# SAP/nested-hashing-psi

Hardware: AMD Instinct MI355X
Metric: server PIE ciphertexts/sec (higher is better)
Workload: dtype u64

## Files before the change

### nested_hashing_psi_amd/csrc/kernels_pie.hip

```cpp
#include <stdlib.h>

#include <cassert>

#include <algorithm>

#include "kernels.hpp"
#include "madasm.h"
#include "stage_a_common.h"
#include "pie_arith.h"

namespace piehip {

static const u32 TPB = 256;

typedef u64 u64x2 __attribute__((ext_vector_type(2)));


template <int BPT>
__global__ void __launch_bounds__(TPB) stage_a_kernel(const DevConsts *__restrict__ dc, u32 N, u32 L, u32 K, u32 b, u32 E,
                                                      const u64 *__restrict__ idx, const u64 *__restrict__ minus,
                                                      const u64 *__restrict__ db, u64 *__restrict__ acc, u32 bstride, u32 h0,
                                                      u32 nq, u32 q)
{
    const u32 n = 2 * (blockIdx.x * TPB + threadIdx.x);
    const u32 l = blockIdx.y;
    const u32 groups = b / BPT;
    const u32 h = h0 + blockIdx.z / groups, beta0 = (blockIdx.z % groups) * BPT;
    if (n >= N) return;
    const Mod m = dc->mod[l];
    const size_t LN = (size_t)L * N;
    const u64 *pi = idx + ((size_t)h * E) * 2 * LN + (size_t)l * N + n;
    const u64 *pd = db + (((size_t)h * bstride + beta0) * E) * LN + (size_t)l * N + n;
    const size_t bin_stride = (size_t)E * LN;
    U128 a[BPT][2][2];
#pragma unroll
    for (int t = 0; t < BPT; t++)
#pragma unroll
        for (int c = 0; c < 2; c++) a[t][c][0] = a[t][c][1] = U128{0, 0};
    for (u32 j = 0; j < E; j++) {
        const u64x2 i0 = *reinterpret_cast<const u64x2 *>(pi + (size_t)j * 2 * LN);
        const u64x2 i1 = *reinterpret_cast<const u64x2 *>(pi + (size_t)j * 2 * LN + LN);
        u64x2 d[BPT];
#pragma unroll
        for (int t = 0; t < BPT; t++) {
            typedef u64 u64v2 __attribute__((ext_vector_type(2)));
            const u64v2 v = __builtin_nontemporal_load(reinterpret_cast<const u64v2 *>(pd + (size_t)t * bin_stride + (size_t)j * LN));
            d[t].x = v.x, d[t].y = v.y;
        }
#pragma unroll
        for (int t = 0; t < BPT; t++) {
            mac128(a[t][0][0], i0.x, d[t].x);
            mac128(a[t][0][1], i0.y, d[t].y);
            mac128(a[t][1][0], i1.x, d[t].x);
            mac128(a[t][1][1], i1.y, d[t].y);
        }
        if ((j & 31) == 31) {
#pragma unroll
            for (int t = 0; t < BPT; t++)
#pragma unroll
                for (int c = 0; c < 2; c++)
#pragma unroll
                    for (int e = 0; e < 2; e++) a[t][c][e] = U128{reduce128(a[t][c][e], m), 0};
        }
    }
    const u64x2 m0 = *reinterpret_cast<const u64x2 *>(minus + (size_t)l * N + n);
    const u64x2 m1 = *reinterpret_cast<const u64x2 *>(minus + LN + (size_t)l * N + n);
#pragma unroll
    for (int t = 0; t < BPT; t++) {
        u64 *po = acc + ((((size_t)(beta0 + t) * nq + q) * K + h) * 2) * LN + (size_t)l * N + n;
        u64x2 r0, r1;
        r0.x = addmod(reduce128(a[t][0][0], m), m0.x, m.q);
        r0.y = addmod(reduce128(a[t][0][1], m), m0.y, m.q);
        r1.x = addmod(reduce128(a[t][1][0], m), m1.x, m.q);
        r1.y = addmod(reduce128(a[t][1][1], m), m1.y, m.q);
        *reinterpret_cast<u64x2 *>(po) = r0;
        *reinterpret_cast<u64x2 *>(po + LN) = r1;
    }
}

static const int SA_DEPTH = 4;
template <int BPT>
__global__ void __launch_bounds__(TPB) stage_a_mad_kernel(const DevConsts *__restrict__ dc, u32 N, u32 L, u32 K, u32 b, u32 E,
                                                          const u64 *__restrict__ idx, const u64 *__restrict__ minus,
                                                          const u64 *__restrict__ db, u64 *__restrict__ acc, u32 bstride, u32 h0,
                                                          u32 nq, u32 q, StageAXOut xo)
{
    const u32 nl = threadIdx.x;
    const u32 n = blockIdx.x * TPB + nl;
    const u32 l = blockIdx.y;
    const u32 groups = b / BPT;
    const u32 h = h0 + blockIdx.z / groups, beta0 = (blockIdx.z % groups) * BPT;
    if (n >= N) return;
    const Mod m = dc->mod[l];
    const size_t LN = (size_t)L * N;
    const u64 *pi = idx + ((size_t)h * E) * 2 * LN + (size_t)l * N + blockIdx.x * TPB;
    const u64 *pd = db + (((size_t)h * bstride + beta0) * E) * LN + (size_t)l * N + blockIdx.x * TPB;
    const size_t bin_stride = (size_t)E * LN;
    ColAcc a[BPT][2];
#pragma unroll
    for (int t = 0; t < BPT; t++) a[t][0] = a[t][1] = ColAcc{0, 0, 0};
    auto load_term = [&](u32 j, u64 (&vi)[2], u64 (&vd)[BPT]) {
        const u64 *pij = pi + (size_t)j * 2 * LN, *pdj = pd + (size_t)j * LN;
        vi[0] = pij[nl];
        vi[1] = (pij + LN)[nl];
#pragma unroll
        for (int t = 0; t < BPT; t++) vd[t] = __builtin_nontemporal_load(pdj + (size_t)t * bin_stride + nl);
    };
    u64 qiv[SA_DEPTH][2], qdv[SA_DEPTH][BPT];
#pragma unroll
    for (int d = 0; d < SA_DEPTH; d++)
        if ((u32)d < E) load_term(d, qiv[d], qdv[d]);
    auto term = [&](u32 j, u64 (&vi)[2], u64 (&vd)[BPT]) {
        const Split30 i0 = split30(vi[0]), i1 = split30(vi[1]);
#pragma unroll
        for (int t = 0; t < BPT; t++) colacc_mac2(a[t][0], a[t][1], i0, i1, vd[t]);
        if (j + SA_DEPTH < E) load_term(j + SA_DEPTH, vi, vd);
        if ((j % COLACC_MAX_TERMS) == COLACC_MAX_TERMS - 1 && j + 1 < E) {
#pragma unroll
            for (int t = 0; t < BPT; t++) colacc_carry(a[t][0]), colacc_carry(a[t][1]);
        }
        if ((j % COLACC_MAX_TOTAL) == COLACC_MAX_TOTAL - 1 && j + 1 < E) {
#pragma unroll
            for (int t = 0; t < BPT; t++)
#pragma unroll
                for (int c = 0; c < 2; c++) {
                    const u64 r = reduce124(colacc_value(a[t][c]), m);
                    a[t][c] = ColAcc{r & 0x3FFFFFFFull, r >> 30, 0};
                }
        }
    };
    for (u32 j = 0; j < E; j += SA_DEPTH) {
#pragma unroll
        for (int d = 0; d < SA_DEPTH; d++)
            if (j + d < E) term(j + d, qiv[d], qdv[d]);
    }
    const bool xdir = h == 0 && xo.out != nullptr;
    const u32 noff = n + ((xdir ? ~0u : 0u) & (lane_home(n, xo.logns) - n));
#pragma unroll
    for (int t = 0; t < BPT; t++) {
        const size_t row = (size_t)(beta0 + t) * nq + q;
        u64 *const base = xdir ? xo.out + ((row * 4) * xo.M + l) * N : acc + ((row * K + h) * 2) * LN + (size_t)l * N;
        const size_t cstride = xdir ? (size_t)xo.M * N : LN;
        u64 *const po = base + noff;
#pragma unroll
        for (int c = 0; c < 2; c++)
            po[(size_t)c * cstride] = addmod_nb(colacc_reduce<true>(a[t][c], m, 0 - m.q), minus[(size_t)c * LN + (size_t)l * N + n], m.q);
    }
}

template <int BPT, int Q, int DEPTH>
__global__ void __launch_bounds__(TPB) stage_a_mad_batch_kernel(const DevConsts *__restrict__ dc, u32 N, u32 L, u32 K, u32 b, u32 E,
                                                                StageAQueries qs, const u64 *__restrict__ db, u64 *__restrict__ acc,
                                                                u32 bstride, u32 h0, u32 nq, u32 q0, u32 tiles, StageAXOut xo)
{
    StageATile tl;
    if (!stage_a_tile((N + TPB - 1) / TPB, L, tiles, (b + BPT - 1) / BPT, tl)) return;
    const u32 nl = threadIdx.x, n0 = tl.bx * TPB, l = tl.l, h = h0 + tl.hz, beta0 = tl.grp * BPT;
    const u32 n = n0 + nl;
    if (n >= N) return;
    const u32 tmax = __builtin_amdgcn_readfirstlane(min((u32)BPT, b - beta0) - 1);
    const Mod m = dc->mod[l];
    const size_t LN = (size_t)L * N;
    const size_t ioff = ((size_t)h * E) * 2 * LN + (size_t)l * N + n0;
    const u64 *pd = db + (((size_t)h * bstride + beta0) * E) * LN + (size_t)l * N + n0;
    const size_t bin_stride = (size_t)E * LN;
    StageAAcc<true> a[Q][BPT][2];
    stage_a_terms<BPT, Q, DEPTH, true>(qs, ioff, LN, pd, bin_stride, tmax, nl, E, m, a);
    const bool xdir = h == 0 && xo.out != nullptr;
    const u32 noff = n + ((xdir ? ~0u : 0u) & (lane_home(n, xo.logns) - n));
#pragma unroll
    for (int q = 0; q < Q; q++) {
        u64 mi[2];
#pragma unroll
        for (int c = 0; c < 2; c++) mi[c] = qs.minus[q][(size_t)c * LN + (size_t)l * N + n];
#pragma unroll
        for (int t = 0; t < BPT; t++) {
            if ((u32)t > tmax) continue;
            const size_t row = (size_t)(beta0 + t) * nq + q0 + q;
            u64 *const base = xdir ? xo.out + ((row * 4) * xo.M + l) * N : acc + ((row * K + h) * 2) * LN + (size_t)l * N;
            const size_t cstride = xdir ? (size_t)xo.M * N : LN;
            u64 *const po = base + noff;
#pragma unroll
            for (int c = 0; c < 2; c++) po[(size_t)c * cstride] = addmod_nb(colacc_reduce<true>(a[q][t][c].v, m, 0 - m.q), mi[c], m.q);
        }
    }
}

static void launch_stage_a_uniform(const DevConsts *dc, u32 N, u32 L, u32 K, u32 b, u32 E, const u64 *idx, const u64 *minus,
                                   const u64 *db, u64 *acc, hipStream_t st, bool mad, u32 bstride, u32 h0, u32 hn, int bpt, u32 nq,
                                   u32 q, StageAXOut xo)
{
    const int cpt = mad ? 1 : 2;
    dim3 grid((N / cpt + TPB - 1) / TPB, L, hn * (b / bpt));
#define SA(B_)                                                                                                       \
    do {                                                                                                             \
        if (mad) hipLaunchKernelGGL(stage_a_mad_kernel<B_>, grid, dim3(TPB), 0, st, dc, N, L, K, b, E, idx, minus, db, acc, bstride, h0, nq, q, xo); \
        else hipLaunchKernelGGL(stage_a_kernel<B_>, grid, dim3(TPB), 0, st, dc, N, L, K, b, E, idx, minus, db, acc, bstride, h0, nq, q);  \
    } while (0)
    switch (bpt) {
        case 8: hipLaunchKernelGGL(stage_a_kernel<8>, grid, dim3(TPB), 0, st, dc, N, L, K, b, E, idx, minus, db, acc, bstride, h0, nq, q); break;
        case 7: SA(7); break;
        case 6: SA(6); break;
        case 5: SA(5); break;
        case 4: SA(4); break;
        case 3: SA(3); break;
        case 2: SA(2); break;
        default: SA(1); break;
    }
#undef SA
}

void launch_stage_a(const DevConsts *dc, u32 N, u32 L, u32 K, u32 b, u32 E, const u64 *idx, const u64 *minus,
                    const u64 *db, u64 *acc, hipStream_t st, bool small_moduli, u32 bstride, u32 h0, u32 hn, u32 nq, u32 q,
                    const StageAXOut *xop)
{
    StageAXOut xo;
    if (xop && small_moduli) xo = *xop;
    if (!bstride) bstride = b;
    if (!hn) hn = K - h0;
    if (!nq) nq = 1;
    const bool mad = small_moduli;
    const u32 cap = mad ? 7 : 8;
    u32 bpt = 0;
    for (u32 c = cap; c >= 4; c--)
        if (b % c == 0) {
            bpt = c;
            break;
        }
    if (b <= cap) bpt = b;
    const size_t LN = (size_t)L * N;
    if (bpt) {
        launch_stage_a_uniform(dc, N, L, K, b, E, idx, minus, db, acc, st, mad, bstride, h0, hn, (int)bpt, nq, q, xo);
        return;
    }
    const u32 full = (b / cap) * cap, rest = b - full;
    launch_stage_a_uniform(dc, N, L, K, full, E, idx, minus, db, acc, st, mad, bstride, h0, hn, (int)cap, nq, q, xo);
    StageAXOut xr = xo;
    if (xr.out) xr.out += (size_t)full * nq * 4 * xr.M * N;
    launch_stage_a_uniform(dc, N, L, K, rest, E, idx, minus, db + (size_t)full * E * LN, acc + (size_t)full * nq * K * 2 * LN, st, mad,
                           bstride, h0, hn, (int)rest, nq, q, xr);
}

template <int Q, int BPT>
static void launch_stage_a_batch_qb(const DevConsts *dc, u32 N, u32 L, u32 K, u32 nb, u32 E, const StageAQueries &qs, const u64 *db,
                                    u64 *acc, hipStream_t st, u32 bstride, u32 h0, u32 hn, u32 nq, u32 q0, StageAXOut xo)
{
    const u32 nx = (N + TPB - 1) / TPB;
    constexpr int DEPTH = stage_a_depth(Q, BPT);
    hipLaunchKernelGGL((stage_a_mad_batch_kernel<BPT, Q, DEPTH>), stage_a_grid(nx, L, hn, (nb + BPT - 1) / BPT), dim3(TPB), 0, st, dc, N, L, K,
                       nb, E, qs, db, acc, bstride, h0, nq, q0, nx * L * hn, xo);
}
template <int Q>
static void launch_stage_a_batch_q(const DevConsts *dc, u32 N, u32 L, u32 K, u32 b, u32 E, const StageAQueries &qs, const u64 *db,
                                   u64 *acc, hipStream_t st, u32 bstride, u32 h0, u32 hn, u32 nq, u32 q0, StageAXOut xo)
{
    constexpr u32 cap = stage_a_layer_cap(Q, true);
    const u32 bpt = stage_a_layers(Q, b, cap);
    if constexpr (cap >= 4)
        if (bpt == 4) return launch_stage_a_batch_qb<Q, 4>(dc, N, L, K, b, E, qs, db, acc, st, bstride, h0, hn, nq, q0, xo);
    if constexpr (cap >= 3)
        if (bpt == 3) return launch_stage_a_batch_qb<Q, 3>(dc, N, L, K, b, E, qs, db, acc, st, bstride, h0, hn, nq, q0, xo);
    if (bpt == 2) return launch_stage_a_batch_qb<Q, 2>(dc, N, L, K, b, E, qs, db, acc, st, bstride, h0, hn, nq, q0, xo);
    return launch_stage_a_batch_qb<Q, 1>(dc, N, L, K, b, E, qs, db, acc, st, bstride, h0, hn, nq, q0, xo);
}
void launch_stage_a_batch(const DevConsts *dc, u32 N, u32 L, u32 K, u32 b, u32 E, const StageAQueries &qs, u32 nq, const u64 *db,
                          u64 *acc, hipStream_t st, bool small_moduli, u32 bstride, u32 h0, u32 hn, const StageAXOut *xop)
{
    StageAXOut xo;
    if (xop && small_moduli) xo = *xop;
    if (!bstride) bstride = b;
    if (!hn) hn = K - h0;
    u32 q0 = 0;
    while (small_moduli && nq - q0 >= 2) {
        const u32 g = stage_a_query_group(nq - q0);
        StageAQueries sub = {};
        for (u32 q = 0; q < g; q++) sub.idx[q] = qs.idx[q0 + q], sub.minus[q] = qs.minus[q0 + q];
        if (g == 2) launch_stage_a_batch_q<2>(dc, N, L, K, b, E, sub, db, acc, st, bstride, h0, hn, nq, q0, xo);
        else if (g == 3) launch_stage_a_batch_q<3>(dc, N, L, K, b, E, sub, db, acc, st, bstride, h0, hn, nq, q0, xo);
        else launch_stage_a_batch_q<4>(dc, N, L, K, b, E, sub, db, acc, st, bstride, h0, hn, nq, q0, xo);
        q0 += g;
    }
    for (; q0 < nq; q0++)
        launch_stage_a(dc, N, L, K, b, E, qs.idx[q0], qs.minus[q0], db, acc, st, small_moduli, bstride, h0, hn, nq, q0, xop);
}

#define PIE_ITER_FENCE() __builtin_amdgcn_sched_barrier(0)
typedef const __attribute__((address_space(4))) DevConsts *DcC;
__device__ __forceinline__ DcC dc_iter(const DevConsts *dc)
{
    u64 v = (u64)dc;
    asm volatile("" : "+s"(v));
    return (DcC)v;
}
__device__ __forceinline__ Mod ld_mod(DcC c, u32 i)
{
    Mod m;
    m.q = c->mod[i].q, m.r0 = c->mod[i].r0, m.r1 = c->mod[i].r1, m.n_inv = 0, m.n_inv_sh = 0;
    m.fconst = c->mod[i].fconst, m.fshift = c->mod[i].fshift, m.pad = 0;
    return m;
}

__device__ __forceinline__ void fold_load(const DevConsts *dc, u32 a, u64 u, u64 v, u64 &x0, u64 &x1)
{
    PIE_ITER_FENCE();
    const DcC c = dc_iter(dc);
    const u64 q = c->mod[a].q, nq = neg_u(q);
    x0 = shoup63(u + v, c->fold_ia[a], c->fold_ia_sh[a], nq);
    x1 = shoup63(u + (4 * q - v), c->fold_ib[a], c->fold_ib_sh[a], nq);
}
__device__ __forceinline__ void fold_store(const DevConsts *dc, u32 a, u64 u, u64 v, u64 &y0, u64 &y1)
{
    const DcC c = dc_iter(dc);
    const u64 q = c->mod[a].q;
    const u64 t = shoup63_lazy(v, c->fold_w[a], c->fold_w_sh[a], neg_u(q));
    y0 = u + t;
    y1 = u + (4 * q - t);
}

template <u32 L, bool MAD, bool YIN, int NP, bool LZ = false>
__device__ __forceinline__ void expand_core(const DevConsts *dc, const u64 (&x)[NP][L], u64 (&out)[NP][2 * L + 1])
{
    constexpr u32 Lp = L + 1;
    u64 y[NP][L];
    u64 fsum[NP];
#pragma unroll
    for (int p = 0; p < NP; p++) fsum[p] = 0;
#pragma unroll
    for (u32 i = 0; i < L; i++) {
        PIE_ITER_FENCE();
        const DcC c = dc_iter(dc);
        const Mod mi = ld_mod(c, i);
        const u64 w = c->qhat_inv[i], wsh = c->qhat_inv_sh[i], nq = neg_u(mi.q);
#pragma unroll
        for (int p = 0; p < NP; p++) {
            out[p][i] = x[p][i];
            y[p][i] = YIN ? x[p][i] : mshoup<MAD>(x[p][i], w, wsh, mi.q, nq);
            fsum[p] += mfixfrac<MAD>(y[p][i], mi);
        }
    }
#pragma unroll
    for (u32 j = 0; j < Lp; j++) {
        PIE_ITER_FENCE();
        const DcC c = dc_iter(dc);
        const Mod pj = ld_mod(c, L + j);
        u64 hat[L];
#pragma unroll
        for (u32 i = 0; i < L; i++) hat[i] = c->qhat_modp[i][j];
        const u64 prodmod = c->Q_modp[j], nq = neg_u(pj.q), n2q = neg_u(2 * pj.q);
#pragma unroll
        for (int p = 0; p < NP; p++) out[p][L + j] = crt_out<L, MAD, LZ>(y[p], hat, (fsum[p] + FIX_HALF) >> 60, prodmod, pj, nq, n2q);
    }
}

template <u32 L, bool MAD, bool YIN, int NP, bool LZ = false>
__device__ __forceinline__ void scale_pq_core(const DevConsts *dc, const u64 (&x)[NP][L], u64 (&out)[NP][2 * L + 1])
{
    constexpr u32 Lp = L + 1;
    u64 y[NP][L];
    u64 fsum[NP];
    U128 itot[NP];
#pragma unroll
    for (int p = 0; p < NP; p++) fsum[p] = 0, itot[p] = U128{0, 0};
#pragma unroll
    for (u32 i = 0; i < L; i++) {
        PIE_ITER_FENCE();
        const DcC c = dc_iter(dc);
        const Mod mi = ld_mod(c, i);
        const u64 w = c->qhat_inv[i], wsh = c->qhat_inv_sh[i], pw = c->P_modq[i], pwsh = c->P_modq_sh[i], nq = neg_u(mi.q);
#pragma unroll
        for (int p = 0; p < NP; p++) {
            y[p][i] = YIN ? x[p][i] : mshoup<MAD>(x[p][i], w, wsh, mi.q, nq);
            u64 fl, z;
            mdivmod<MAD>(y[p][i], pw, pwsh, mi.q, nq, fl, z);
            add128(itot[p], U128{fl, 0});
            fsum[p] += mfixfrac<MAD>(z, mi);
        }
    }
    u64 yp[NP][Lp];
    u64 fs2[NP];
#pragma unroll
    for (int p = 0; p < NP; p++) {
        add128(itot[p], U128{(fsum[p] + FIX_HALF) >> 60, 0});
        fs2[p] = 0;
    }
#pragma unroll
    for (u32 j = 0; j < Lp; j++) {
        PIE_ITER_FENCE();
        const DcC c = dc_iter(dc);
        const Mod pj = ld_mod(c, L + j);
        u64 col[L];
#pragma unroll
        for (u32 i = 0; i < L; i++) col[i] = c->PI_modp[i][j];
        const u64 w = c->phat_inv[j], wsh = c->phat_inv_sh[j], nq = neg_u(pj.q);
#pragma unroll
        for (int p = 0; p < NP; p++) {
            u64 r;
            if (MAD) {
                ColAcc a = {itot[p].lo, 0, 0};
#pragma unroll
                for (u32 i = 0; i < L; i++) colacc_mac(a, split30(y[p][i]), split30(col[i]));
                r = LZ ? colacc_reduce123_lazy(a, pj, nq) : colacc_reduce<false>(a, pj, nq);
            } else {
                U128 acc = dot128<L, MAD>(y[p], col);
                add128(acc, itot[p]);
                r = reduce128(acc, pj);
            }
            out[p][L + j] = r;
            yp[p][j] = mshoup<MAD>(r, w, wsh, pj.q, nq);
            fs2[p] += mfixfrac<MAD>(yp[p][j], pj);
        }
    }
#pragma unroll
    for (u32 i = 0; i < L; i++) {
        PIE_ITER_FENCE();
        const DcC c = dc_iter(dc);
        const Mod mi = ld_mod(c, i);
        u64 hat[Lp];
#pragma unroll
        for (u32 j = 0; j < Lp; j++) hat[j] = c->phat_modq[j][i];
        const u64 prodmod = c->P_modq[i], nq = neg_u(mi.q), n2q = neg_u(2 * mi.q);
#pragma unroll
        for (int p = 0; p < NP; p++) out[p][i] = crt_out<Lp, MAD, LZ>(yp[p], hat, (fs2[p] + FIX_HALF) >> 60, prodmod, mi, nq, n2q);
    }
}

template <bool SCALE, bool FOLD, u32 L, bool MAD, bool SKIPQ>
__device__ __forceinline__ void expand_body(const DevConsts *__restrict__ dc, u32 N, const u64 *__restrict__ in, size_t so, size_t si,
                                            u64 *__restrict__ out, u32 out_polys, u32 out_slot, u32 by)
{
    constexpr bool YIN = FOLD && (SCALE || SKIPQ);
    const u32 n = blockIdx.x * TPB + threadIdx.x;
    const u32 H = N / 2;
    if (n >= (FOLD ? H : N)) return;
    const u32 o = by >> 1, c = by & 1;
    constexpr u32 M = 2 * L + 1;
    const u64 *pin = in + (size_t)o * so + (size_t)c * si + n;
    u64 *pout = out + ((size_t)(o * out_polys + out_slot + c) * M) * N + n;
    constexpr int NP = FOLD ? 2 : 1;
    u64 x[NP][L], y[NP][M];
#pragma unroll
    for (u32 i = 0; i < L; i++) {
        if (YIN) {
            PIE_ITER_FENCE();
            const DcC c = dc_iter(dc);
            const u64 q = c->mod[i].q, nq = neg_u(q), u = pin[(size_t)i * N], v = pin[(size_t)i * N + H];
            x[0][i] = shoup63(u + v, c->fold_iaq[i], c->fold_iaq_sh[i], nq);
            x[NP - 1][i] = shoup63(u + (4 * q - v), c->fold_ibq[i], c->fold_ibq_sh[i], nq);
        } else if (FOLD) {
            fold_load(dc, i, pin[(size_t)i * N], pin[(size_t)i * N + H], x[0][i], x[NP - 1][i]);
        } else {
            x[0][i] = pin[(size_t)i * N];
        }
    }
    constexpr bool LZ = FOLD && MAD;
    if (SCALE)
        scale_pq_core<L, MAD, YIN, NP, LZ>(dc, x, y);
    else
        expand_core<L, MAD, YIN, NP, LZ>(dc, x, y);
#pragma unroll
    for (u32 a = 0; a < M; a++) {
        if (!SCALE && a < L && SKIPQ) continue;
        PIE_ITER_FENCE();
        if (FOLD) {
            u64 y0, y1;
            fold_store(dc, a, y[0][a], y[NP - 1][a], y0, y1);
            pout[(size_t)a * N] = y0;
            pout[(size_t)a * N + H] = y1;
        } else {
            pout[(size_t)a * N] = y[0][a];
        }
    }
}

template <bool SCALE, bool FOLD, u32 L, bool MAD, bool SKIPQ>
__global__ void __launch_bounds__(TPB) expand_kernel(const DevConsts *__restrict__ dc, u32 N, const u64 *__restrict__ in,
                                                     size_t so, size_t si, u64 *__restrict__ out, u32 out_polys, u32 out_slot)
{
    expand_body<SCALE, FOLD, L, MAD, SKIPQ>(dc, N, in, so, si, out, out_polys, out_slot, blockIdx.y);
}
template <bool FOLD, u32 L, bool MAD, bool SKIPQ>
__global__ void __launch_bounds__(TPB) expand_both_kernel(const DevConsts *__restrict__ dc, u32 N, const u64 *__restrict__ x, size_t sx,
                                                          const u64 *__restrict__ y, size_t sy, size_t si, u64 *__restrict__ out,
                                                          u32 n_outer)
{
    if (blockIdx.y < 2 * n_outer)
        expand_body<true, FOLD, L, MAD, false>(dc, N, y, sy, si, out, 4, 2, blockIdx.y);
    else
        expand_body<false, FOLD, L, MAD, SKIPQ>(dc, N, x, sx, si, out, 4, 0, blockIdx.y - 2 * n_outer);
}
void launch_expand_both(const DevConsts *dc, u32 N, u32 L, const u64 *x, size_t sx, const u64 *y, size_t sy, size_t si, u32 n_outer,
                        u64 *out, hipStream_t st, bool small_moduli, bool fold, bool skip_q)
{
    dim3 grid(((fold ? N / 2 : N) + TPB - 1) / TPB, n_outer * 4);
#define EB(F_, L_, M_, Q_) hipLaunchKernelGGL((expand_both_kernel<F_, L_, M_, Q_>), grid, dim3(TPB), 0, st, dc, N, x, sx, y, sy, si, out, n_outer)
#define EBL(L_)                                                                          \
    case L_:                                                                             \
        if (fold && small_moduli) { if (skip_q) EB(true, L_, true, true); else EB(true, L_, true, false); }      \
        else if (fold) { if (skip_q) EB(true, L_, false, true); else EB(true, L_, false, false); }                 \
        else if (small_moduli) { if (skip_q) EB(false, L_, true, true); else EB(false, L_, true, false); }       \
        else { if (skip_q) EB(false, L_, false, true); else EB(false, L_, false, false); }                         \
        break;
    switch (L) { EBL(1) EBL(2) EBL(3) EBL(4) EBL(5) EBL(6) EBL(7) }
#undef EBL
#undef EB
}

static void launch_expand_common(bool scale, bool fold, const DevConsts *dc, u32 N, u32 L, const u64 *in, size_t so, size_t si,
                                 u32 n_outer, u64 *out, u32 out_polys, u32 out_slot, hipStream_t st, bool small_moduli, bool skip_q = false)
{
    dim3 grid(((fold ? N / 2 : N) + TPB - 1) / TPB, n_outer * 2);
#define EX(S_, F_, L_, Q_)                                                                                                    \
    do {                                                                                                                      \
        if (small_moduli)                                                                                                   \
            hipLaunchKernelGGL((expand_kernel<S_, F_, L_, true, Q_>), grid, dim3(TPB), 0, st, dc, N, in, so, si, out, out_polys, out_slot); \
        else                                                                                                                  \
            hipLaunchKernelGGL((expand_kernel<S_, F_, L_, false, Q_>), grid, dim3(TPB), 0, st, dc, N, in, so, si, out, out_polys, out_slot); \
    } while (0)
#define EXL(L_)                                                         \
    case L_:                                                            \
        if (scale) {                                                    \
            if (fold) EX(true, true, L_, false); else EX(true, false, L_, false); \
        } else if (skip_q) {                                            \
            if (fold) EX(false, true, L_, true); else EX(false, false, L_, true); \
        } else {                                                        \
            if (fold) EX(false, true, L_, false); else EX(false, false, L_, false); \
        }                                                               \
        break;
    switch (L) { EXL(1) EXL(2) EXL(3) EXL(4) EXL(5) EXL(6) EXL(7) }
#undef EXL
#undef EX
}
void launch_expand_q_to_qp(const DevConsts *dc, u32 N, u32 L, const u64 *in, size_t so, size_t si, u32 n_outer, u64 *out,
                           u32 out_polys, u32 out_slot, hipStream_t st, bool small_moduli, bool fold, bool skip_q)
{
    launch_expand_common(false, fold, dc, N, L, in, so, si, n_outer, out, out_polys, out_slot, st, small_moduli, skip_q);
}
void launch_scale_pq_expand(const DevConsts *dc, u32 N, u32 L, const u64 *in, size_t so, size_t si, u32 n_outer, u64 *out,
                            u32 out_polys, u32 out_slot, hipStream_t st, bool small_moduli, bool fold)
{
    launch_expand_common(true, fold, dc, N, L, in, so, si, n_outer, out, out_polys, out_slot, st, small_moduli);
}

template <bool MAD>
__global__ void __launch_bounds__(TPB) tensor_kernel(const DevConsts *dc, u32 N, u32 M, const u64 *__restrict__ e,
                                                     u64 *__restrict__ d)
{
    const u32 n = 2 * (blockIdx.x * TPB + threadIdx.x);
    if (n >= N) return;
    const u32 a = blockIdx.y, bin = blockIdx.z;
    const Mod m = dc->mod[a];
    const size_t MN = (size_t)M * N;
    const u64 *pe = e + (size_t)bin * 4 * MN + (size_t)a * N + n;
    u64 *pd = d + (size_t)bin * 3 * MN + (size_t)a * N + n;
    const u64x2 va0 = *reinterpret_cast<const u64x2 *>(pe), va1 = *reinterpret_cast<const u64x2 *>(pe + MN),
                vb0 = *reinterpret_cast<const u64x2 *>(pe + 2 * MN), vb1 = *reinterpret_cast<const u64x2 *>(pe + 3 * MN);
    u64x2 r0, r1, r2;
#pragma unroll
    for (int k = 0; k < 2; k++) {
        u64 a0 = k ? va0.y : va0.x, a1 = k ? va1.y : va1.x, b0 = k ? vb0.y : vb0.x, b1 = k ? vb1.y : vb1.x;
        u64 d0, d1, d2;
        if (MAD) {
            const u64 nq = neg_u(m.q), n2q = neg_u(2 * m.q), n4q = neg_u(4 * m.q);
            a0 = csub_u(csub_u(a0, n4q), n2q), a1 = csub_u(csub_u(a1, n4q), n2q);
            b0 = csub_u(csub_u(b0, n4q), n2q), b1 = csub_u(csub_u(b1, n4q), n2q);
            const Split30 sa0 = split30(a0), sa1 = split30(a1), sb0 = split30(b0), sb1 = split30(b1);
            ColAcc c = {0, 0, 0};
            colacc_mac(c, sa0, sb0);
            d0 = colacc_reduce<false>(c, m, nq);
            c = ColAcc{0, 0, 0};
            colacc_mac(c, sa0, sb1);
            colacc_mac(c, sa1, sb0);
            d1 = colacc_reduce<false>(c, m, nq);
            c = ColAcc{0, 0, 0};
            colacc_mac(c, sa1, sb1);
            d2 = colacc_reduce<false>(c, m, nq);
        } else {
            d0 = mulmod(a0, b0, m);
            U128 x = mul128(a0, b1);
            mac128(x, a1, b0);
            d1 = reduce128(x, m);
            d2 = mulmod(a1, b1, m);
// ... 596 lines not shown
```

### nested_hashing_psi_amd/csrc/stage_a_common.h

```cpp
#pragma once
#include "kernels.hpp"
#include "madasm.h"

namespace piehip {

#define PIE_ASM_CLOB "vcc", "v60", "v61", "v62", "v63", "v64", "v65", "v66", "v67", "v68", "v69", "v70", "v71"

struct StageATile {
    u32 bx, l, hz, grp;
};
__device__ __forceinline__ bool stage_a_tile(u32 nx, u32 L, u32 tiles, u32 groups, StageATile &t)
{
    const u32 id = blockIdx.x, xcd = id & 7, slot = id >> 3;
    t.grp = slot % groups;
    const u32 tile = (slot / groups) * 8 + xcd;
    if (tile >= tiles) return false;
    t.bx = tile % nx;
    t.l = (tile / nx) % L;
    t.hz = tile / (nx * L);
    return true;
}
static dim3 stage_a_grid(u32 nx, u32 L, u32 hn, u32 groups) { return dim3(8 * ((nx * L * hn + 7) / 8) * groups); }

__device__ __forceinline__ u32 lane_home(u32 n, u32 logns)
{
    const u32 ns = 1u << logns, e = n & (ns - 1);
    return (n & ~(ns - 1)) + 2 * ((ns >> 4) * ((e >> 1) & 7) + (e >> 4)) + (e & 1);
}

__device__ __forceinline__ u64 addmod_nb(u64 a, u64 b, u64 q)
{
    const u64 s = a + b;
    u32 lo, hi;
    asm("v_lshl_add_u64 v[60:61], %[x], 0, %[nm]\n\t"
        "v_ashrrev_i32 v62, 31, v61\n\t"
        "v_bfi_b32 %[lo], v62, %[xl], v60\n\t"
        "v_bfi_b32 %[hi], v62, %[xh], v61"
        : [lo] "=&v"(lo), [hi] "=&v"(hi)
        : [x] "v"(s), [xl] "v"((u32)s), [xh] "v"((u32)(s >> 32)), [nm] "s"(0 - q)
        : "v62", "v60", "v61");
    return ((u64)hi << 32) | lo;
}

#define PIE_COLACC123_TO_4Q \
    "v_lshrrev_b64 v[60:61], 30, %[c0]\n\t" \
    "v_lshl_add_u64 v[60:61], v[60:61], 0, %[c1]\n\t" \
    "v_lshrrev_b64 v[62:63], 30, v[60:61]\n\t" \
    "v_lshl_add_u64 v[62:63], v[62:63], 0, %[c2]\n\t" \
    "v_lshlrev_b64 v[64:65], 1, v[62:63]\n\t" \
    "v_bfe_u32 v68, v60, 29, 1\n\t" \
    "v_and_b32 v66, 0x3fffffff, %[c0l]\n\t" \
    "v_bfe_u32 v67, v60, 2, 28\n\t" \
    "v_or_b32 v64, v64, v68\n\t" \
    "v_lshl_or_b32 v66, v60, 30, v66\n\t" \
    "v_lshl_or_b32 v67, v62, 28, v67\n\t" \
    "v_mul_hi_u32 v68, v64, %[mul]\n\t" \
    "v_mov_b32 v69, 0\n\t" \
    "v_mad_u64_u32 v[68:69], vcc, v64, %[muh], v[68:69]\n\t" \
    "v_mad_u64_u32 v[68:69], vcc, v65, %[mul], v[68:69]\n\t" \
    "v_mad_u64_u32 v[70:71], s[96:97], v65, %[muh], 0\n\t" \
    "v_lshrrev_b64 v[68:69], 32, v[68:69]\n\t" \
    "v_addc_co_u32 v69, vcc, 0, v69, vcc\n\t" \
    "v_lshl_add_u64 v[68:69], v[70:71], 0, v[68:69]\n\t" \
    "v_mad_u64_u32 v[70:71], vcc, v68, %[nqh], 0\n\t" \
    "v_mad_u64_u32 v[70:71], vcc, v69, %[nql], v[70:71]\n\t" \
    "v_add_u32 v67, v67, v70\n\t" \
    "v_mad_u64_u32 v[66:67], vcc, v68, %[nql], v[66:67]\n\t"
__device__ __forceinline__ u64 colacc_reduce123_lazy(const ColAcc &a, const Mod &m, u64 nq)
{
    const u64 mu = (m.r1 << 59) | (m.r0 >> 5);
    u64 r;
    asm(PIE_COLACC123_TO_4Q
        "v_lshl_add_u64 %[r], v[66:67], 0, 0"
        : [r] "=v"(r)
        : [c0] "v"(a.c0), [c1] "v"(a.c1), [c2] "v"(a.c2), [c0l] "v"((u32)a.c0), [mul] "s"((u32)mu), [muh] "s"((u32)(mu >> 32)),
          [nql] "s"((u32)nq), [nqh] "s"((u32)(nq >> 32))
        : PIE_ASM_CLOB, "s96", "s97");
    return r;
}
template <bool W124>
__device__ __forceinline__ u64 colacc_reduce(const ColAcc &a, const Mod &m, u64 nq)
{
    const u64 mu = (m.r1 << 59) | (m.r0 >> 5);
    const u64 n2q = 2 * nq, n4q = 4 * nq;
    u64 r;
    if (!W124) {
        asm(PIE_COLACC123_TO_4Q
            "v_lshl_add_u64 v[60:61], v[66:67], 0, %[n2q]\n\t"
            "v_ashrrev_i32 v62, 31, v61\n\t"
            "v_bfi_b32 v66, v62, v66, v60\n\t"
            "v_bfi_b32 v67, v62, v67, v61\n\t"
            "v_lshl_add_u64 v[60:61], v[66:67], 0, %[n1q]\n\t"
            "v_ashrrev_i32 v62, 31, v61\n\t"
            "v_and_b32 v64, %[ql], v62\n\t"
            "v_and_b32 v65, %[qh], v62\n\t"
            "v_lshl_add_u64 %[r], v[60:61], 0, v[64:65]"
            : [r] "=v"(r)
            : [c0] "v"(a.c0), [c1] "v"(a.c1), [c2] "v"(a.c2), [c0l] "v"((u32)a.c0), [mul] "s"((u32)mu), [muh] "s"((u32)(mu >> 32)),
              [nql] "s"((u32)nq), [nqh] "s"((u32)(nq >> 32)), [n2q] "s"(n2q), [n1q] "s"(nq), [ql] "s"((u32)m.q), [qh] "s"((u32)(m.q >> 32))
            : PIE_ASM_CLOB, "s96", "s97");
    } else {
        asm("v_lshrrev_b64 v[60:61], 30, %[c0]\n\t"
            "v_lshl_add_u64 v[60:61], v[60:61], 0, %[c1]\n\t"
            "v_lshrrev_b64 v[64:65], 30, v[60:61]\n\t"
            "v_lshl_add_u64 v[64:65], v[64:65], 0, %[c2]\n\t"
            "v_and_b32 v66, 0x3fffffff, %[c0l]\n\t"
            "v_bfe_u32 v67, v60, 2, 28\n\t"
            "v_lshl_or_b32 v66, v60, 30, v66\n\t"
            "v_lshl_or_b32 v67, v64, 28, v67\n\t"
            "v_mul_hi_u32 v68, v64, %[mul]\n\t"
            "v_mov_b32 v69, 0\n\t"
            "v_mad_u64_u32 v[68:69], vcc, v64, %[muh], v[68:69]\n\t"
            "v_mad_u64_u32 v[68:69], vcc, v65, %[mul], v[68:69]\n\t"
            "v_mad_u64_u32 v[70:71], s[96:97], v65, %[muh], 0\n\t"
            "v_lshrrev_b64 v[68:69], 32, v[68:69]\n\t"
            "v_addc_co_u32 v69, vcc, 0, v69, vcc\n\t"
            "v_lshl_add_u64 v[68:69], v[70:71], 0, v[68:69]\n\t"
            "v_lshlrev_b64 v[68:69], 1, v[68:69]\n\t"
            "v_mad_u64_u32 v[70:71], vcc, v68, %[nqh], 0\n\t"
            "v_mad_u64_u32 v[70:71], vcc, v69, %[nql], v[70:71]\n\t"
            "v_add_u32 v67, v67, v70\n\t"
            "v_mad_u64_u32 v[66:67], vcc, v68, %[nql], v[66:67]\n\t"
            "v_lshl_add_u64 v[60:61], v[66:67], 0, %[n4q]\n\t"
            "v_ashrrev_i32 v62, 31, v61\n\t"
            "v_bfi_b32 v66, v62, v66, v60\n\t"
            "v_bfi_b32 v67, v62, v67, v61\n\t"
            "v_lshl_add_u64 v[60:61], v[66:67], 0, %[n2q]\n\t"
            "v_ashrrev_i32 v62, 31, v61\n\t"
            "v_bfi_b32 v66, v62, v66, v60\n\t"
            "v_bfi_b32 v67, v62, v67, v61\n\t"
            "v_lshl_add_u64 v[60:61], v[66:67], 0, %[n1q]\n\t"
            "v_ashrrev_i32 v62, 31, v61\n\t"
            "v_and_b32 v64, %[ql], v62\n\t"
            "v_and_b32 v65, %[qh], v62\n\t"
            "v_lshl_add_u64 %[r], v[60:61], 0, v[64:65]"
            : [r] "=v"(r)
            : [c0] "v"(a.c0), [c1] "v"(a.c1), [c2] "v"(a.c2), [c0l] "v"((u32)a.c0), [mul] "s"((u32)mu), [muh] "s"((u32)(mu >> 32)),
              [nql] "s"((u32)nq), [nqh] "s"((u32)(nq >> 32)), [n4q] "s"(n4q), [n2q] "s"(n2q), [n1q] "s"(nq), [ql] "s"((u32)m.q),
              [qh] "s"((u32)(m.q >> 32))
            : PIE_ASM_CLOB, "s96", "s97");
    }
    return r;
}

template <bool MAD>
struct StageAAcc;
template <>
struct StageAAcc<true> {
    ColAcc v;
    __device__ __forceinline__ void zero() { v = ColAcc{0, 0, 0}; }
};
template <>
struct StageAAcc<false> {
    U128 v;
    __device__ __forceinline__ void zero() { v = U128{0, 0}; }
};

template <int BPT, int Q, int DEPTH, bool MAD, class S>
__device__ __forceinline__ void stage_a_terms(const StageAQueries &qs, size_t ioff, S cs, const u64 *pd, size_t bin_stride, u32 tmax, u32 nl,
                                              u32 E, const Mod &m, StageAAcc<MAD> (&out)[Q][BPT][2])
{
    StageAAcc<MAD> a[Q][BPT][2];
#pragma unroll
    for (int q = 0; q < Q; q++)
#pragma unroll
        for (int t = 0; t < BPT; t++) a[q][t][0].zero(), a[q][t][1].zero();
    auto load_term = [&](u32 j, u64 (&vi)[Q][2], u64 (&vd)[BPT]) {
#pragma unroll
        for (int q = 0; q < Q; q++) {
            const u64 *pij = qs.idx[q] + ioff + (size_t)j * 2 * cs;
            vi[q][0] = pij[nl];
            vi[q][1] = (pij + cs)[nl];
        }
        const u64 *pdj = pd + (size_t)j * cs;
#pragma unroll
        for (int t = 0; t < BPT; t++) vd[t] = __builtin_nontemporal_load(pdj + (size_t)min((u32)t, tmax) * bin_stride + nl);
    };
    u64 qiv[DEPTH][Q][2], qdv[DEPTH][BPT];
#pragma unroll
    for (int d = 0; d < DEPTH; d++)
        if ((u32)d < E) load_term(d, qiv[d], qdv[d]);
    auto term = [&](u32 j, u64 (&vi)[Q][2], u64 (&vd)[BPT]) {
#pragma unroll
        for (int q = 0; q < Q; q++) {
            if constexpr (MAD) {
                const Split30 i0 = split30(vi[q][0]), i1 = split30(vi[q][1]);
#pragma unroll
                for (int t = 0; t < BPT; t++) colacc_mac2(a[q][t][0].v, a[q][t][1].v, i0, i1, vd[t]);
            } else {
#pragma unroll
                for (int t = 0; t < BPT; t++) mac128(a[q][t][0].v, vi[q][0], vd[t]), mac128(a[q][t][1].v, vi[q][1], vd[t]);
            }
        }
        if (j + DEPTH < E) load_term(j + DEPTH, vi, vd);
        if constexpr (MAD) {
            if ((j % COLACC_MAX_TERMS) == COLACC_MAX_TERMS - 1 && j + 1 < E) {
#pragma unroll
                for (int q = 0; q < Q; q++)
#pragma unroll
                    for (int t = 0; t < BPT; t++) colacc_carry(a[q][t][0].v), colacc_carry(a[q][t][1].v);
            }
            if ((j % COLACC_MAX_TOTAL) == COLACC_MAX_TOTAL - 1 && j + 1 < E) {
#pragma unroll
                for (int q = 0; q < Q; q++)
#pragma unroll
                    for (int t = 0; t < BPT; t++)
#pragma unroll
                        for (int c = 0; c < 2; c++) {
                            const u64 r = colacc_reduce<true>(a[q][t][c].v, m, 0 - m.q);
                            a[q][t][c].v = ColAcc{r & 0x3FFFFFFFull, r >> 30, 0};
                        }
            }
        } else {
            if ((j & 31) == 31) {
#pragma unroll
                for (int q = 0; q < Q; q++)
#pragma unroll
                    for (int t = 0; t < BPT; t++)
#pragma unroll
                        for (int c = 0; c < 2; c++) a[q][t][c].v = U128{reduce128(a[q][t][c].v, m), 0};
            }
        }
    };
    for (u32 j = 0; j < E; j += DEPTH) {
#pragma unroll
        for (int d = 0; d < DEPTH; d++)
            if (j + d < E) term(j + d, qiv[d], qdv[d]);
    }
#pragma unroll
    for (int q = 0; q < Q; q++)
#pragma unroll
        for (int t = 0; t < BPT; t++) out[q][t][0] = a[q][t][0], out[q][t][1] = a[q][t][1];
}

constexpr u32 stage_a_query_group(u32 left) { return left == 5 || left == 6 ? 3 : left < 4 ? left : 4; }
static_assert(stage_a_query_group(5) == 3 && stage_a_query_group(5 - 3) == 2, "five queries: 3 + 2");
static_assert(stage_a_query_group(7) == 4 && stage_a_query_group(7 - 4) == 3, "seven queries: 4 + 3");

constexpr u32 stage_a_layer_cap(u32 Q, bool mad) { return Q == 1 ? (mad ? 7 : 5) : Q == 2 ? 4 : 3; }
constexpr u32 stage_a_layers(u32 Q, u32 b, u32 cap)
{
    u32 bpt = 1, best = ~0u;
    for (u32 g = 1; g <= cap && g <= b; g++) {
        const u32 loads = ((b + g - 1) / g) * (2 * Q + g);
        if (loads <= best) best = loads, bpt = g;
    }
    return bpt;
}
static_assert(stage_a_layers(2, 6, stage_a_layer_cap(2, true)) == 3, "six layers of two queries: 3 + 3");
static_assert(stage_a_layers(3, 12, stage_a_layer_cap(3, true)) == 3, "twelve layers of three queries: groups of three");

constexpr int stage_a_depth(int Q, int BPT) { return Q == 1 ? (BPT == 7 ? 3 : 4) : (Q == 4 || Q * BPT >= 9) ? 2 : 3; }
}
```

Baseline: 78720.

## Add resident stage-A kernel keeping query indices in registers across all layers

Adds a stage-A kernel for three-query groups with E of 12 or 14. It loads the split query index columns and minus terms into registers once, then loops over every layer of the partition. Database words stream through a nontemporal ring of loads, and the multiply-accumulate is a fused inline-asm block of eight mads. The aim is to stop reloading query data for each small layer group, at the cost of high register pressure and a grid with fewer, longer-running blocks.

```diff
diff --git a/nested_hashing_psi_amd/csrc/kernels_pie.hip b/nested_hashing_psi_amd/csrc/kernels_pie.hip
--- a/nested_hashing_psi_amd/csrc/kernels_pie.hip
+++ b/nested_hashing_psi_amd/csrc/kernels_pie.hip
@@ -183,6 +183,75 @@
 #pragma unroll
             for (int c = 0; c < 2; c++) po[(size_t)c * cstride] = addmod_nb(colacc_reduce<true>(a[q][t][c].v, m, 0 - m.q), mi[c], m.q);
         }
+    }
+}
+
+template <int Q, int E, int D>
+__global__ void __launch_bounds__(TPB) stage_a_resident_kernel(const DevConsts *__restrict__ dc, u32 N, u32 L, u32 K, u32 b, u32 lpp,
+                                                               StageAQueries qs, const u64 *__restrict__ db, u64 *__restrict__ acc,
+                                                               u32 bstride, u32 h0, u32 nq, u32 q0, u32 tiles, StageAXOut xo)
+{
+    static_assert(E % D == 0 && E >= 1 && (u32)E < COLACC_MAX_TOTAL && (u32)E <= 2 * COLACC_MAX_TERMS, "ring slots and sweep periods");
+    StageATile tl;
+    if (!stage_a_tile((N + TPB - 1) / TPB, L, tiles, (b + lpp - 1) / lpp, tl)) return;
+    const u32 nl = threadIdx.x, n0 = tl.bx * TPB, l = tl.l, h = h0 + tl.hz, beta0 = tl.grp * lpp;
+    const u32 n = n0 + nl;
+    if (n >= N) return;
+    const u32 nlay = __builtin_amdgcn_readfirstlane(min(lpp, b - beta0));
+    const Mod m = dc->mod[l];
+    const size_t LN = (size_t)L * N;
+    const size_t ioff = ((size_t)h * E) * 2 * LN + (size_t)l * N + n0;
+    const u64 *pw = db + (((size_t)h * bstride + beta0) * E) * LN + (size_t)l * N + n0;
+    u32 left = nlay * E - 1;
+    u64 r[D];
+#pragma unroll
+    for (int d = 0; d < D; d++) {
+        r[d] = __builtin_nontemporal_load(pw + nl);
+        pw += left ? LN : 0, left -= left ? 1 : 0;
+    }
+    Split30 ix[Q][E][2];
+    u64 mi[Q][2];
+#pragma unroll
+    for (int q = 0; q < Q; q++) {
+#pragma unroll
+        for (int j = 0; j < E; j++)
+#pragma unroll
+            for (int c = 0; c < 2; c++) ix[q][j][c] = split30((qs.idx[q] + ioff + (size_t)(2 * j + c) * LN)[nl]);
+#pragma unroll
+        for (int c = 0; c < 2; c++) mi[q][c] = qs.minus[q][(size_t)c * LN + (size_t)l * N + n];
+    }
+    const bool xdir = h == 0 && xo.out != nullptr;
+    const u32 noff = n + ((xdir ? ~0u : 0u) & (lane_home(n, xo.logns) - n));
+    const size_t cstride = xdir ? (size_t)xo.M * N : LN;
+    for (u32 t = 0; t < nlay; t++) {
+        ColAcc a[Q][2];
+#pragma unroll
+        for (int j = 0; j < E; j++) {
+            const u64 d = r[j % D];
+            const u32 dl = (u32)d & 0x3FFFFFFFu, dh = (u32)(d >> 30);
+            r[j % D] = __builtin_nontemporal_load(pw + nl);
+            pw += left ? LN : 0, left -= left ? 1 : 0;
+            PIE_STAGE_A_FENCE();
+#pragma unroll
+            for (int q = 0; q < Q; q++) {
+                if (j == 0) colacc_mac2_cut<true>(a[q][0], a[q][1], ix[q][j][0], ix[q][j][1], dl, dh);
+                else colacc_mac2_cut<false>(a[q][0], a[q][1], ix[q][j][0], ix[q][j][1], dl, dh);
+            }
+            if (j == (int)COLACC_MAX_TERMS - 1 && j + 1 < E) {
+#pragma unroll
+                for (int q = 0; q < Q; q++) colacc_carry(a[q][0]), colacc_carry(a[q][1]);
+            }
+            PIE_STAGE_A_FENCE();
+        }
+#pragma unroll
+        for (int q = 0; q < Q; q++) {
+            const size_t row = (size_t)(beta0 + t) * nq + q0 + q;
+            u64 *const base = xdir ? xo.out + ((row * 4) * xo.M + l) * N : acc + ((row * K + h) * 2) * LN + (size_t)l * N;
+            u64 *const po = base + noff;
+#pragma unroll
+            for (int c = 0; c < 2; c++) po[(size_t)c * cstride] = addmod_nb(colacc_reduce<true>(a[q][c], m, 0 - m.q), mi[q][c], m.q);
+        }
+        PIE_STAGE_A_FENCE();
     }
 }
 
@@ -263,6 +332,14 @@
     if (bpt == 2) return launch_stage_a_batch_qb<Q, 2>(dc, N, L, K, b, E, qs, db, acc, st, bstride, h0, hn, nq, q0, xo);
     return launch_stage_a_batch_qb<Q, 1>(dc, N, L, K, b, E, qs, db, acc, st, bstride, h0, hn, nq, q0, xo);
 }
+template <int E>
+static void launch_stage_a_resident(const DevConsts *dc, u32 N, u32 L, u32 K, u32 b, u32 lpp, const StageAQueries &qs, const u64 *db,
+                                    u64 *acc, hipStream_t st, u32 bstride, u32 h0, u32 hn, u32 nq, u32 q0, StageAXOut xo)
+{
+    const u32 nx = (N + TPB - 1) / TPB;
+    hipLaunchKernelGGL((stage_a_resident_kernel<3, E, stage_a_resident_ring(E)>), stage_a_grid(nx, L, hn, (b + lpp - 1) / lpp), dim3(TPB), 0, st,
+                       dc, N, L, K, b, lpp, qs, db, acc, bstride, h0, nq, q0, nx * L * hn, xo);
+}
 void launch_stage_a_batch(const DevConsts *dc, u32 N, u32 L, u32 K, u32 b, u32 E, const StageAQueries &qs, u32 nq, const u64 *db,
                           u64 *acc, hipStream_t st, bool small_moduli, u32 bstride, u32 h0, u32 hn, const StageAXOut *xop)
 {
@@ -276,7 +353,12 @@
         StageAQueries sub = {};
         for (u32 q = 0; q < g; q++) sub.idx[q] = qs.idx[q0 + q], sub.minus[q] = qs.minus[q0 + q];
         if (g == 2) launch_stage_a_batch_q<2>(dc, N, L, K, b, E, sub, db, acc, st, bstride, h0, hn, nq, q0, xo);
-        else if (g == 3) launch_stage_a_batch_q<3>(dc, N, L, K, b, E, sub, db, acc, st, bstride, h0, hn, nq, q0, xo);
+        else if (g == 3) {
+            const u32 lpp = stage_a_resident_lpp(3, E, b, (u64)N * L * hn);
+            if (lpp && E == 14) launch_stage_a_resident<14>(dc, N, L, K, b, lpp, sub, db, acc, st, bstride, h0, hn, nq, q0, xo);
+            else if (lpp && E == 12) launch_stage_a_resident<12>(dc, N, L, K, b, lpp, sub, db, acc, st, bstride, h0, hn, nq, q0, xo);
+            else launch_stage_a_batch_q<3>(dc, N, L, K, b, E, sub, db, acc, st, bstride, h0, hn, nq, q0, xo);
+        }
         else launch_stage_a_batch_q<4>(dc, N, L, K, b, E, sub, db, acc, st, bstride, h0, hn, nq, q0, xo);
         q0 += g;
     }
diff --git a/nested_hashing_psi_amd/csrc/stage_a_common.h b/nested_hashing_psi_amd/csrc/stage_a_common.h
--- a/nested_hashing_psi_amd/csrc/stage_a_common.h
+++ b/nested_hashing_psi_amd/csrc/stage_a_common.h
@@ -233,6 +233,37 @@
         for (int t = 0; t < BPT; t++) out[q][t][0] = a[q][t][0], out[q][t][1] = a[q][t][1];
 }
 
+#define PIE_STAGE_A_FENCE() __builtin_amdgcn_sched_barrier(0)
+template <bool FIRST>
+__device__ __forceinline__ void colacc_mac2_cut(ColAcc &a, ColAcc &b, Split30 x0, Split30 x1, u32 dl, u32 dh)
+{
+    if (FIRST) {
+        asm("v_mad_u64_u32 %[a0], vcc, %[x0l], %[dl], 0\n\t"
+            "v_mad_u64_u32 %[a1], vcc, %[x0l], %[dh], 0\n\t"
+            "v_mad_u64_u32 %[b0], vcc, %[x1l], %[dl], 0\n\t"
+            "v_mad_u64_u32 %[b1], vcc, %[x1l], %[dh], 0\n\t"
+            "v_mad_u64_u32 %[a2], vcc, %[x0h], %[dh], 0\n\t"
+            "v_mad_u64_u32 %[b2], vcc, %[x1h], %[dh], 0\n\t"
+            "v_mad_u64_u32 %[a1], vcc, %[x0h], %[dl], %[a1]\n\t"
+            "v_mad_u64_u32 %[b1], vcc, %[x1h], %[dl], %[b1]\n\t"
+            : [a0] "=&v"(a.c0), [a1] "=&v"(a.c1), [a2] "=&v"(a.c2), [b0] "=&v"(b.c0), [b1] "=&v"(b.c1), [b2] "=&v"(b.c2)
+            : [dl] "v"(dl), [dh] "v"(dh), [x0l] "v"(x0.lo), [x0h] "v"(x0.hi), [x1l] "v"(x1.lo), [x1h] "v"(x1.hi)
+            : "vcc");
+    } else {
+        asm("v_mad_u64_u32 %[a0], vcc, %[x0l], %[dl], %[a0]\n\t"
+            "v_mad_u64_u32 %[a1], vcc, %[x0l], %[dh], %[a1]\n\t"
+            "v_mad_u64_u32 %[b0], vcc, %[x1l], %[dl], %[b0]\n\t"
+            "v_mad_u64_u32 %[b1], vcc, %[x1l], %[dh], %[b1]\n\t"
+            "v_mad_u64_u32 %[a2], vcc, %[x0h], %[dh], %[a2]\n\t"
+            "v_mad_u64_u32 %[b2], vcc, %[x1h], %[dh], %[b2]\n\t"
+            "v_mad_u64_u32 %[a1], vcc, %[x0h], %[dl], %[a1]\n\t"
+            "v_mad_u64_u32 %[b1], vcc, %[x1h], %[dl], %[b1]\n\t"
+            : [a0] "+v"(a.c0), [a1] "+v"(a.c1), [a2] "+v"(a.c2), [b0] "+v"(b.c0), [b1] "+v"(b.c1), [b2] "+v"(b.c2)
+            : [dl] "v"(dl), [dh] "v"(dh), [x0l] "v"(x0.lo), [x0h] "v"(x0.hi), [x1l] "v"(x1.lo), [x1h] "v"(x1.hi)
+            : "vcc");
+    }
+}
+
 constexpr u32 stage_a_query_group(u32 left) { return left == 5 || left == 6 ? 3 : left < 4 ? left : 4; }
 static_assert(stage_a_query_group(5) == 3 && stage_a_query_group(5 - 3) == 2, "five queries: 3 + 2");
 static_assert(stage_a_query_group(7) == 4 && stage_a_query_group(7 - 4) == 3, "seven queries: 4 + 3");
@@ -251,4 +282,24 @@
 static_assert(stage_a_layers(3, 12, stage_a_layer_cap(3, true)) == 3, "twelve layers of three queries: groups of three");
 
 constexpr int stage_a_depth(int Q, int BPT) { return Q == 1 ? (BPT == 7 ? 3 : 4) : (Q == 4 || Q * BPT >= 9) ? 2 : 3; }
-}
+
+#ifndef PIEHIP_STAGE_A_RESIDENT
+#define PIEHIP_STAGE_A_RESIDENT 1
+#endif
+constexpr int stage_a_resident_ring(u32 E) { return E == 14 ? 7 : E == 12 ? 6 : 0; }
+constexpr u64 STAGE_A_RESIDENT_MIN_THREADS = 65536;
+constexpr u32 stage_a_resident_lpp(u32 Q, u32 E, u32 b, u64 threads)
+{
+    if (!PIEHIP_STAGE_A_RESIDENT || Q != 3 || !stage_a_resident_ring(E) || b <= stage_a_layer_cap(3, true)) return 0;
+    return threads >= STAGE_A_RESIDENT_MIN_THREADS ? b : 0;
+}
+#if PIEHIP_STAGE_A_RESIDENT
+static_assert(stage_a_resident_lpp(3, 14, 14, 16384 * 4 * 2) == 14 && stage_a_resident_lpp(3, 14, 8, 16384 * 4 * 2) == 8 &&
+                  stage_a_resident_lpp(3, 14, 6, 16384 * 4 * 2) == 6,
+              "C3, three queries: resident on one queue (14 layers) and on two (8 + 6), one partition each");
+#endif
+static_assert(stage_a_resident_lpp(3, 15, 14, 16384 * 4 * 2) == 0 && stage_a_resident_lpp(4, 14, 14, 16384 * 4 * 2) == 0 &&
+                  stage_a_resident_lpp(3, 14, 3, 16384 * 4 * 2) == 0 && stage_a_resident_lpp(2, 14, 14, 16384 * 4 * 2) == 0,
+              "E = 15, four or two queries and a launch of one layer group stay on the tiled kernel");
+static_assert(stage_a_resident_lpp(3, 12, 12, 8192 * 3 * 2) == 0, "C2 stays on the tiled kernel (under one wave per SIMD)");
+}
```

New measurement: 80570 (median of 6 runs). 1.02x the previous value.
